# GlaireDaggers/Pretty-Fast-Video

Measured on AMD Instinct MI355X. Metric: macroblocks/s (encode+decode) 1080p YUV420, higher is better.
Workload: dtype i32 (encoder transforms evaluated in exact f32; decoders i32)

## Files before the change

### pretty-fast-video_amd/csrc/pfv_device.h

```cpp
#pragma once
#include <stdint.h>

#ifdef PFV_HIPEMU
#define PFV_WAVES_PER_EU(n)
#else
#define PFV_WAVES_PER_EU(n) __attribute__((amdgpu_waves_per_eu(n, n)))
#endif

namespace pfv {

constexpr int kStripMB = 8;
#ifndef PFV_STRIPS_PER_WG
#define PFV_STRIPS_PER_WG 4
#endif
constexpr int kStripsPerWG = PFV_STRIPS_PER_WG;
constexpr int kThreads = 64 * kStripsPerWG;

struct QTab {
    float rcp[64];
    int32_t deq[64];
};

struct PlaneGeom {
    int w, h;
    int pw, ph;
    int bw, bh;
    int strips_x;
    int strip0;
    int tiles_y;
    int tile0;
    int mb0;
    int qsel;
    int clear;
    int fast_src;
    long src_off;
    long pad_off;
};

struct FrameGeom {
    PlaneGeom p[3];
    int n_planes;
    int strips_per_frame;
    int tiles_per_frame;
    int mbs_per_frame;
    int n_streams;
    long src_frame_bytes;
    long pad_frame_bytes;
    const uint8_t *const *src_slots;
};
__host__ __device__ inline const uint8_t *frame_src(const FrameGeom &g, const uint8_t *src, int stream)
{
    return g.src_slots ? g.src_slots[stream] : src + (long)stream * g.src_frame_bytes;
}

struct CoefLists {
    const uint32_t *const *entries;
    const uint32_t *counts;
};
constexpr uint32_t coef_entry(uint32_t mb, uint32_t pos, int16_t value) { return ((uint32_t)(uint16_t)value << 16) | ((mb & 255u) << 8) | (pos & 255u); }

}
```

### pretty-fast-video_amd/csrc/pfv_kernels.hip

```cpp
#include <hip/hip_runtime.h>
#include <stdint.h>

#include "pfv_device.h"
#include "pfv_prof.h"


namespace pfv {

namespace {
__constant__ int kScale[64] = {
    32, 37, 34, 26, 32, 26, 34, 37, 37, 43, 39, 31, 37, 31, 39, 43, 34, 39, 35, 28, 34, 28, 35, 39, 26, 31, 28, 22, 26, 22,
    28, 31, 32, 37, 34, 26, 32, 26, 34, 37, 26, 31, 28, 22, 26, 22, 28, 31, 34, 39, 35, 28, 34, 28, 35, 39, 37, 43, 39, 31,
    37, 31, 39, 43,
};
__constant__ int kInvZigzag[64] = {
    0,  1,  5,  6,  14, 15, 27, 28, 2,  4,  7,  13, 16, 26, 29, 42, 3,  8,  12, 17, 25, 30, 41, 43, 9,  11, 18, 24, 31, 40,
    44, 53, 10, 19, 23, 32, 39, 45, 52, 54, 20, 22, 33, 38, 46, 51, 55, 60, 21, 34, 37, 47, 50, 56, 59, 61, 35, 36, 48, 49,
    57, 58, 62, 63,
};
}

constexpr int kWinRows = 16 * kStripsPerWG + 30;
constexpr int kWinStride = 176;
constexpr int kWinBytes = kWinRows * kWinStride;
// ... 137 lines not shown
    int a5 = wadd(wadd(wsub(b5.x, b6.x), b6.q), b6.s);
    int a6 = wsub(wsub(wadd(b6.x, b5.x), b5.q), b5.s);
    int a0 = wadd(b0, b2), a1 = wadd(b1, b3), a2 = wsub(b1, b3), a3 = wsub(b0, b2);
    v[0] = wadd(a0, a4); v[1] = wadd(a1, a5); v[2] = wadd(a2, a6); v[3] = wadd(a3, a7);
    v[4] = wsub(a3, a7); v[5] = wsub(a2, a6); v[6] = wsub(a1, a5); v[7] = wsub(a0, a4);
}

__device__ __forceinline__ void rows_to_cols2(int (&v)[2][8], int *mb, int i, int mx)
{
    const int sw = (i >> 2) & 1;
#pragma unroll
    for (int s = 0; s < 2; s++) {
        int4 *w = reinterpret_cast<int4 *>(mb + s * 64 + (i ^ mx) * 8);
        w[sw] = make_int4(v[s][0], v[s][1], v[s][2], v[s][3]);
        w[sw ^ 1] = make_int4(v[s][4], v[s][5], v[s][6], v[s][7]);
    }
    wave_lds_sync();
    const int lo = i, hi = i ^ 4;
#pragma unroll
    for (int s = 0; s < 2; s++) {
#pragma unroll
        for (int r = 0; r < 8; r++) v[s][r] = mb[s * 64 + (r ^ mx) * 8 + (r < 4 ? lo : hi)];
    }
    wave_lds_sync();
}
__device__ __forceinline__ void cols_to_rows2(int (&v)[2][8], int *mb, int i, int mx)
{
    const int lo = i, hi = i ^ 4;
#pragma unroll
    for (int s = 0; s < 2; s++) {
#pragma unroll
        for (int r = 0; r < 8; r++) mb[s * 64 + (r ^ mx) * 8 + (r < 4 ? lo : hi)] = v[s][r];
    }
    wave_lds_sync();
    const int sw = (i >> 2) & 1;
#pragma unroll
    for (int s = 0; s < 2; s++) {
        const int4 *w = reinterpret_cast<const int4 *>(mb + s * 64 + (i ^ mx) * 8);
        int4 a = w[sw], b = w[sw ^ 1];
        v[s][0] = a.x; v[s][1] = a.y; v[s][2] = a.z; v[s][3] = a.w;
        v[s][4] = b.x; v[s][5] = b.y; v[s][6] = b.z; v[s][7] = b.w;
    }
    wave_lds_sync();
}

struct LaneQ {
    const int *tab;
    int c;
    __device__ __forceinline__ float rcp(int k) const { return __int_as_float(tab[(k * 8 + c) * 4 + 0]); }
    __device__ __forceinline__ int scale(int k) const { return tab[(k * 8 + c) * 4 + 1]; }
    __device__ __forceinline__ int zz(int k) const { return tab[(k * 8 + c) * 4 + 2]; }
    __device__ __forceinline__ int deq(int k) const { return tab[(k * 8 + c) * 4 + 3]; }
    __device__ __forceinline__ float deqf(int k) const { return __int_as_float(tab[(k * 8 + c) * 4 + 3]); }
};
constexpr int kQTabDwords = 4 * 64;
template <bool ENC, bool FLT = false>
__device__ __forceinline__ int4 load_qentry(const QTab *qt, int lane)
{
    int4 e;
    e.x = ENC ? __float_as_int(qt->rcp[lane]) : 0;
    e.y = ENC ? (FLT ? (kScale[lane] << 16) : kScale[lane]) : 0;
    e.z = kInvZigzag[lane];
    e.w = FLT ? __float_as_int((float)qt->deq[lane]) : qt->deq[lane];
    return e;
}
template <bool ENC, bool FLT = false>
__device__ __forceinline__ void fill_qtable(int *tab, const QTab *qt, int lane)
{
    reinterpret_cast<int4 *>(tab)[lane] = load_qentry<ENC, FLT>(qt, lane);
}
__device__ __forceinline__ unsigned pack4(int a, int b, int c, int d)
{
    return (unsigned)a | ((unsigned)b << 8) | ((unsigned)c << 16) | ((unsigned)d << 24);
}
__device__ __forceinline__ int byte_of(unsigned w, int i) { return (int)((w >> (8 * i)) & 0xffu); }

__device__ __forceinline__ void unpack_row(const uint4 &row, int (&px)[2][8])
{
#pragma unroll
    for (int k = 0; k < 4; k++) {
        px[0][k] = byte_of(row.x, k); px[0][k + 4] = byte_of(row.y, k);
        px[1][k] = byte_of(row.z, k); px[1][k + 4] = byte_of(row.w, k);
    }
}
__device__ __forceinline__ uint4 pack_row(const int (&px)[2][8])
{
    return make_uint4(pack4(px[0][0], px[0][1], px[0][2], px[0][3]), pack4(px[0][4], px[0][5], px[0][6], px[0][7]),
                      pack4(px[1][0], px[1][1], px[1][2], px[1][3]), pack4(px[1][4], px[1][5], px[1][6], px[1][7]));
}

__device__ __forceinline__ uint4 ld_stream(const uint4 *p)
{
    return make_uint4(__builtin_nontemporal_load(&p->x), __builtin_nontemporal_load(&p->y), __builtin_nontemporal_load(&p->z),
                      __builtin_nontemporal_load(&p->w));
}
__device__ __forceinline__ void st_stream(uint4 *p, const uint4 &v)
{
    __builtin_nontemporal_store(v.x, &p->x); __builtin_nontemporal_store(v.y, &p->y);
    __builtin_nontemporal_store(v.z, &p->z); __builtin_nontemporal_store(v.w, &p->w);
}

__device__ __forceinline__ uint4 load_src16(const uint8_t *plane, const PlaneGeom &p, int x, int y)
{
    unsigned fill = (unsigned)p.clear * 0x01010101u;
    uint4 val = make_uint4(fill, fill, fill, fill);
    if (y < p.h && x < p.w) {
        const uint8_t *src = plane + (long)y * p.w + x;
        if (p.fast_src && x + 16 <= p.w) {
            val = *reinterpret_cast<const uint4 *>(src);
        } else {
            unsigned wds[4];
#pragma unroll
            for (int i = 0; i < 4; i++) {
                unsigned acc = 0;
#pragma unroll
                for (int b = 0; b < 4; b++) {
                    int xx = x + i * 4 + b;
                    unsigned px = xx < p.w ? (unsigned)src[i * 4 + b] : (unsigned)p.clear;
                    acc |= px << (8 * b);
                }
                wds[i] = acc;
            }
            val = make_uint4(wds[0], wds[1], wds[2], wds[3]);
        }
    }
    return val;
}

__device__ __forceinline__ uint4 load_unaligned16(const uint8_t *p)
{
    int sh = (int)((uintptr_t)p & 3);
    const unsigned *d = reinterpret_cast<const unsigned *>(p - sh);
    unsigned d0 = d[0], d1 = d[1], d2 = d[2], d3 = d[3], d4 = sh ? d[4] : 0u;
    return make_uint4(__builtin_amdgcn_alignbyte(d1, d0, sh), __builtin_amdgcn_alignbyte(d2, d1, sh),
                      __builtin_amdgcn_alignbyte(d3, d2, sh), __builtin_amdgcn_alignbyte(d4, d3, sh));
}

__device__ __forceinline__ void store_cropped16(uint8_t *plane, const PlaneGeom &p, int x, int y, const uint4 &val)
{
    if (y < p.h && x < p.w) st_stream(reinterpret_cast<uint4 *>(plane + (long)y * p.w + x), val);
}

typedef __attribute__((address_space(3))) void lds_void_t;
typedef __attribute__((address_space(1))) const void gbl_cvoid_t;

__device__ __forceinline__ int stage_chunk(int ch) { return (ch >> 4) * kStageChunks + (ch & 15); }
__device__ __forceinline__ void store_coef_half(const int *stage, int16_t *coef_mb0, int n_mb, int lane, int h)
{
#pragma unroll
    for (int j = 0; j < 2; j++) {
        int ch = j * 64 + lane;
        int mb = ch >> 4;
        if (mb < n_mb) st_stream(&reinterpret_cast<uint4 *>(coef_mb0)[mb * 32 + h * 16 + (ch & 15)], reinterpret_cast<const uint4 *>(stage)[stage_chunk(ch)]);
    }
}
__device__ __forceinline__ void fetch_coef_half(uint4 (&buf)[2], const int16_t *coef_mb0, int n_mb, int lane, int h)
{
#pragma unroll
    for (int j = 0; j < 2; j++) {
        int ch = j * 64 + lane;
        int mb = ch >> 4;
        buf[j] = make_uint4(0, 0, 0, 0);
        if (mb < n_mb) buf[j] = ld_stream(&reinterpret_cast<const uint4 *>(coef_mb0)[mb * 32 + h * 16 + (ch & 15)]);
    }
}
__device__ __forceinline__ void store_coef_quads(const int *stage, int16_t *coef_mb0, int n_mb, int lane, int half_strip)
{
#pragma unroll
    for (int j = 0; j < 2; j++) {
        int ch = j * 64 + lane;
        int mb = half_strip * 4 + (ch >> 5);
        if (mb < n_mb) st_stream(&reinterpret_cast<uint4 *>(coef_mb0)[half_strip * 128 + ch], reinterpret_cast<const uint4 *>(stage)[stage_chunk(ch)]);
    }
}
__device__ __forceinline__ void fetch_coef_quads(uint4 (&buf)[2], const int16_t *coef_mb0, int n_mb, int lane, int half_strip)
{
#pragma unroll
    for (int j = 0; j < 2; j++) {
        int ch = j * 64 + lane;
        int mb = half_strip * 4 + (ch >> 5);
        buf[j] = make_uint4(0, 0, 0, 0);
        if (mb < n_mb) buf[j] = ld_stream(&reinterpret_cast<const uint4 *>(coef_mb0)[half_strip * 128 + ch]);
    }
}
__device__ __forceinline__ void stage_coef_half(int *stage, const uint4 (&buf)[2], int lane)
{
#pragma unroll
    for (int j = 0; j < 2; j++) reinterpret_cast<uint4 *>(stage)[stage_chunk(j * 64 + lane)] = buf[j];
}

struct ListSpan {
    const uint32_t *ent;
    uint32_t lo, hi;
    uint32_t e0, e1;
};
__device__ __forceinline__ ListSpan list_span(const uint32_t *ent, uint32_t begin, uint32_t end, int last_lane, int lane)
{
    ListSpan sp{ent, 0u, 0u, 0u, 0u};
    sp.lo = (uint32_t)__builtin_amdgcn_readlane((int)begin, 0);
    sp.hi = (uint32_t)__builtin_amdgcn_readlane((int)end, last_lane);
    if (sp.hi < sp.lo) sp.hi = sp.lo;
    const uint32_t k = sp.lo + (uint32_t)lane;
    if (k < sp.hi) sp.e0 = ent[k];
    if (k + 64u < sp.hi) sp.e1 = ent[k + 64u];
    return sp;
}
template <int LPM>
__device__ __forceinline__ void stage_list_put(int16_t *stage, uint32_t e, int mb_low, int h)
{
    const int pos = (int)(e & 255u), mbl = (int)(((e >> 8) - (uint32_t)mb_low) & 255u);
    if (LPM == 8) {
        if ((pos >> 7) == h && mbl < kStripMB) stage[mbl * (2 * kStagePitch) + (pos & 127)] = (int16_t)(e >> 16);
    } else {
        if (mbl < kStripMB / 2) stage[(mbl * 2 + (pos >> 7)) * (2 * kStagePitch) + (pos & 127)] = (int16_t)(e >> 16);
    }
}
template <int LPM>
__device__ __forceinline__ void stage_list_half(int *xw, const ListSpan &sp, int lane, int mb_low, int h)
{
#pragma unroll
    for (int j = 0; j < 2; j++) reinterpret_cast<uint4 *>(xw)[stage_chunk(j * 64 + lane)] = make_uint4(0, 0, 0, 0);
    wave_lds_sync();
    int16_t *stage = reinterpret_cast<int16_t *>(xw);
    const uint32_t k = sp.lo + (uint32_t)lane;
    if (k < sp.hi) stage_list_put<LPM>(stage, sp.e0, mb_low, h);
    if (k + 64u < sp.hi) stage_list_put<LPM>(stage, sp.e1, mb_low, h);
    for (uint32_t j = k + 128u; j < sp.hi; j += 64u) stage_list_put<LPM>(stage, sp.ent[j], mb_low, h);
}

__device__ __forceinline__ void forward_half(int (&v)[2][8], int *xw, int m, int i, const LaneQ &lq, bool keep)
{
    const int keepmask = keep ? -1 : 0;
    int *mb = xw + m * kMBPitch;
    fdct8(v[0]);
    fdct8(v[1]);
// ... 117 lines not shown
        for (int j = 0; j < 4; j++) {
            const float4 c = row[f_chunk(p, j)];
            x[2 * j] = f2{c.x, c.y};
            x[2 * j + 1] = f2{c.z, c.w};
        }
    }
    wave_lds_sync();
}
__device__ __forceinline__ f2 quant_scale(f2 m, int scale16)
{
    f2 n;
#pragma unroll
    for (int s = 0; s < 2; s++) n[s] = (float)mulhi24((int)m[s], scale16);
    return n;
}
constexpr float kQuantMagic = 12582912.0f;
__device__ __forceinline__ f2 quant_div(f2 n, float rcp, float magic, f2 &biased)
{
    const f2 q = f2trunc(n * f2s(rcp));
    biased = q + f2s(magic);
    return q;
}
__device__ __forceinline__ f2 quant_pair_f(f2 m, int scale16, float rcp, float magic, f2 &biased)
{
    return quant_div(quant_scale(m, scale16), rcp, magic, biased);
}
__device__ __forceinline__ f2 residual_f(f2 src, f2 pred)
{
    const f2 d = src - pred;
    const float c = 0.5f - 1.0f / 2048.0f;
    const f2 r = f2{__builtin_fmaf(d[0], c, kQuantMagic), __builtin_fmaf(d[1], c, kQuantMagic)};
    return f2{__builtin_fmaf(r[0], 256.0f, -256.0f * kQuantMagic), __builtin_fmaf(r[1], 256.0f, -256.0f * kQuantMagic)};
}
__device__ __forceinline__ int16_t quant_low16(float biased) { return (int16_t)__float_as_int(biased); }
__device__ __forceinline__ void forward_half_f(f2 (&x)[8], int *xw, int m, int i, const LaneQ &lq, float magic)
{
    int *mb = xw + m * kMBPitch;
    ffdct8(x);
    f_rows_to_cols(x, mb, i, m & 3);
    ffdct8(x);
    int16_t *stage = reinterpret_cast<int16_t *>(xw) + m * (2 * kStagePitch);
#pragma unroll
    for (int k = 0; k < 8; k++) {
        const int zz = lq.zz(k);
        f2 biased;
        x[k] = quant_pair_f(x[k], lq.scale(k), lq.rcp(k), magic, biased);
#pragma unroll
        for (int s = 0; s < 2; s++) stage[s * 64 + zz] = quant_low16(biased[s]);
    }
    wave_lds_sync();
}
constexpr float kPixelBias = 127.501953125f;
__device__ __forceinline__ f2 iframe_pixel_f(f2 x) { return x * f2s(1.0f / 256.0f) + f2s(kPixelBias); }
template <bool PIXEL>
__device__ __forceinline__ void inverse_half_f(f2 (&c)[8], int *xw, int m, int i, const LaneQ &lq)
{
    int *mb = xw + m * kMBPitch;
#pragma unroll
    for (int k = 0; k < 8; k++) c[k] = c[k] * f2s(lq.deqf(k));
    fidct8(c);
    f_cols_to_rows(c, mb, i, m & 3);
    fidct8(c);
#pragma unroll
    for (int k = 0; k < 8; k++) c[k] = PIXEL ? iframe_pixel_f(c[k]) : f2floor(c[k] * f2s(1.0f / 256.0f));
}
__device__ __forceinline__ uint4 pack_row_f(const f2 (&px)[8])
{
    unsigned w[4] = {0, 0, 0, 0};
#pragma unroll
    for (int k = 0; k < 8; k++) {
        w[k >> 2] = __builtin_amdgcn_cvt_pk_u8_f32(px[k][0], (unsigned)(k & 3), w[k >> 2]);
        w[2 + (k >> 2)] = __builtin_amdgcn_cvt_pk_u8_f32(px[k][1], (unsigned)(k & 3), w[2 + (k >> 2)]);
    }
    return make_uint4(w[0], w[1], w[2], w[3]);
}
__device__ __forceinline__ void unpack_row_f(const uint4 &row, f2 (&px)[8])
{
#pragma unroll
    for (int k = 0; k < 4; k++) {
        px[k] = f2{(float)byte_of(row.x, k), (float)byte_of(row.z, k)};
        px[k + 4] = f2{(float)byte_of(row.y, k), (float)byte_of(row.w, k)};
    }
}

template <bool FLT, int LPM = 8>
__global__ __launch_bounds__(kThreads) void k_enc_iframe(FrameGeom g, const uint8_t *__restrict__ src,
                                                          int16_t *__restrict__ coef, uint8_t *__restrict__ recon,
                                                          const QTab *__restrict__ qtabs, float qmagic)
{
    __shared__ __attribute__((aligned(16))) int xchg[kStripsPerWG][kXchgDwords];
    __shared__ __attribute__((aligned(16))) int qtab_lds[kStripsPerWG][kQTabDwords];
    constexpr int kPasses = LPM == 8 ? 2 : 1;

    const int lane = threadIdx.x & 63, wave = __builtin_amdgcn_readfirstlane((int)(threadIdx.x >> 6));
    const int gw = xcd_remap((int)blockIdx.x, (int)gridDim.x) * kStripsPerWG + wave;
    const int gstrip = LPM == 8 ? gw : gw >> 1, half_strip = LPM == 8 ? 0 : gw & 1;
    if (gstrip >= g.strips_per_frame * g.n_streams) return;
    const StripPos sp = locate_strip(g, gstrip);
    if (half_strip * 4 >= sp.n_mb) return;
    const PlaneGeom &p = g.p[sp.plane];
    const int slot = lane >> 3, i = lane & 7;
    const int m = LPM == 8 ? slot : half_strip * 4 + (slot >> 1);
    int *xw = xchg[wave];

    fill_qtable<true, FLT>(qtab_lds[wave], qtabs + p.qsel, lane);
    const uint8_t *plane = frame_src(g, src, sp.stream) + p.src_off;
    uint4 rows[kPasses];
#pragma unroll
    for (int pass = 0; pass < kPasses; pass++) rows[pass] = load_src16(plane, p, sp.x0 + m * 16, sp.y0 + i + 8 * (LPM == 8 ? pass : (slot & 1)));

    wave_lds_sync();
    const LaneQ lq{qtab_lds[wave], i};
    int16_t *coef_mb0 = coef + ((long)sp.stream * g.mbs_per_frame + sp.mb_first) * 256;
    uint8_t *dst = recon ? recon + (long)sp.stream * g.pad_frame_bytes + p.pad_off + (long)(sp.y0 + i) * p.pw + sp.x0 + m * 16
                         : nullptr;
#pragma unroll
    for (int pass = 0; pass < kPasses; pass++) {
        const int h = LPM == 8 ? pass : (slot & 1);
        if (FLT) {
            f2 x[8];
            unpack_row_f(rows[pass], x);
#pragma unroll
            for (int k = 0; k < 8; k++) x[k] = x[k] * f2s(256.0f) - f2s(32768.0f);
            forward_half_f(x, xw, slot, i, lq, qmagic);
            if (LPM == 8) store_coef_half(xw, coef_mb0, sp.n_mb, lane, h);
            else store_coef_quads(xw, coef_mb0, sp.n_mb, lane, half_strip);
            wave_lds_sync();
            if (recon) {
                inverse_half_f<true>(x, xw, slot, i, lq);
                if (m < sp.n_mb) *reinterpret_cast<uint4 *>(dst + (long)(8 * h) * p.pw) = pack_row_f(x);
            }
        } else {
            int v[2][8];
            unpack_row(rows[pass], v);
#pragma unroll
// ... 286 lines not shown
    const int wrow0 = mby - tp.winy0 + i;

    unsigned s2 = 0;
#pragma unroll
    for (int h = 0; h < 2; h++) {
        s2 = __builtin_amdgcn_udot4(rows[h].x, rows[h].x, s2, false);
        s2 = __builtin_amdgcn_udot4(rows[h].y, rows[h].y, s2, false);
        s2 = __builtin_amdgcn_udot4(rows[h].z, rows[h].z, s2, false);
        s2 = __builtin_amdgcn_udot4(rows[h].w, rows[h].w, s2, false);
    }
    const int a2 = mb_sum((int)s2);

    SearchState st;
    st.cx = 0; st.cy = 0; st.err = 0;
    const SearchLane sl = make_search_lane(red, m, i, neg2);
    const bool interior = sp.x0 >= 16 && sp.x0 + kStripMB * 16 + 16 <= p.pw && sp.y0 >= 16 && sp.y0 + 32 <= p.ph;
    if (interior) {
        search_level<8, true, false, DPPRED>(win, wrow0, wcol0, rows[0], rows[1], a2, mbx, mby, p.pw, p.ph, st, sl);
        KMARK(3);
        search_level<4, false, false, DPPRED>(win, wrow0, wcol0, rows[0], rows[1], a2, mbx, mby, p.pw, p.ph, st, sl);
        KMARK(4);
        search_level<2, false, false, DPPRED>(win, wrow0, wcol0, rows[0], rows[1], a2, mbx, mby, p.pw, p.ph, st, sl);
        KMARK(5);
        search_level<1, false, false, DPPRED>(win, wrow0, wcol0, rows[0], rows[1], a2, mbx, mby, p.pw, p.ph, st, sl);
        KMARK(6);
    } else {
        search_level<8, true, true, DPPRED>(win, wrow0, wcol0, rows[0], rows[1], a2, mbx, mby, p.pw, p.ph, st, sl);
        search_level<4, false, true, DPPRED>(win, wrow0, wcol0, rows[0], rows[1], a2, mbx, mby, p.pw, p.ph, st, sl);
        search_level<2, false, true, DPPRED>(win, wrow0, wcol0, rows[0], rows[1], a2, mbx, mby, p.pw, p.ph, st, sl);
        search_level<1, false, true, DPPRED>(win, wrow0, wcol0, rows[0], rows[1], a2, mbx, mby, p.pw, p.ph, st, sl);
    }

    so.coded = mb_valid && !((float)st.err <= min_err);
    so.cx = st.cx; so.cy = st.cy;

    const int wx = wcol0 + st.cx, shp = wx & 3;
    const uint8_t *rp = win + (wrow0 + st.cy) * kWinStride + (wx & ~3);
#pragma unroll
    for (int h = 0; h < 2; h++) {
        const unsigned *d = reinterpret_cast<const unsigned *>(rp + 8 * h * kWinStride);
        unsigned d0 = d[0], d1 = d[1], d2 = d[2], d3 = d[3], d4 = d[4];
        so.patch[h] = make_uint4(__builtin_amdgcn_alignbyte(d1, d0, shp), __builtin_amdgcn_alignbyte(d2, d1, shp),
                                 __builtin_amdgcn_alignbyte(d3, d2, shp), __builtin_amdgcn_alignbyte(d4, d3, shp));
    }
}

__device__ __forceinline__ void opaque_row(uint4 &r)
{
#ifndef PFV_HIPEMU
    asm volatile("" : "+v"(r.x), "+v"(r.y), "+v"(r.z), "+v"(r.w));
#else
    (void)r;
#endif
}
template <bool FLT, bool REUNPACK = false, class Store>
__device__ __forceinline__ uint4 penc_half(const uint4 &srow, const uint4 &prow, int *xw, int m, int i, const LaneQ &lq, float qmagic, bool want_recon,
                                           Store &&store)
{
    uint4 out = prow;
    if (FLT) {
        f2 x[8], pp[8];
        unpack_row_f(srow, x);
        unpack_row_f(prow, pp);
#pragma unroll
        for (int k = 0; k < 8; k++) x[k] = residual_f(x[k], pp[k]);
        forward_half_f(x, xw, m, i, lq, qmagic);
        store();
        wave_lds_sync();
        if (want_recon) {
            inverse_half_f<false>(x, xw, m, i, lq);
            if (REUNPACK) {
                uint4 again = prow;
                opaque_row(again);
                unpack_row_f(again, pp);
            }
#pragma unroll
            for (int k = 0; k < 8; k++) {
                const f2 t = f2{__builtin_fminf(x[k][0], 127.0f), __builtin_fminf(x[k][1], 127.0f)};
                pp[k] = pp[k] + t * f2s(2.0f);
            }
            out = pack_row_f(pp);
        }
    } else {
        int v[2][8], pp[2][8];
        unpack_row(srow, v);
        unpack_row(prow, pp);
#pragma unroll
        for (int s = 0; s < 2; s++) {
#pragma unroll
            for (int k = 0; k < 8; k++) {
                int d = v[s][k] - pp[s][k];
                v[s][k] = (int)((unsigned)tdiv2(d) << 8);
            }
        }
        forward_half(v, xw, m, i, lq, true);
        store();
        wave_lds_sync();
        if (want_recon) {
            inverse_half(v, xw, m, i, lq);
#pragma unroll
            for (int s = 0; s < 2; s++) {
#pragma unroll
                for (int k = 0; k < 8; k++)
                    pp[s][k] = min(max(pp[s][k] + 2 * v[s][k], 0), 255);
            }
            out = pack_row(pp);
// ... 515 lines not shown
        if (recon && mb_valid) *reinterpret_cast<uint4 *>(dst) = o;
    } else if (mb_valid) {
        uint4 *cm = reinterpret_cast<uint4 *>(coef_mb0 + m * 256);
        st_stream(&cm[r], make_uint4(0, 0, 0, 0));
        st_stream(&cm[16 + r], make_uint4(0, 0, 0, 0));
        if (dst) *reinterpret_cast<uint4 *>(dst) = patch;
    }
}

template <int LPM = 8, bool LISTS = false>
__global__ __launch_bounds__(kThreads) void k_dec_iframe(FrameGeom g, const int16_t *__restrict__ coef, CoefLists cl,
                                                          uint8_t *__restrict__ out, const QTab *__restrict__ qtabs,
                                                          uint8_t *__restrict__ frames_out)
{
    __shared__ __attribute__((aligned(16))) int xchg[kStripsPerWG][kXchgDwords];
    __shared__ __attribute__((aligned(16))) int qtab_lds[kStripsPerWG][kQTabDwords];
    constexpr int kPasses = LPM == 8 ? 2 : 1;

    const int lane = threadIdx.x & 63, wave = __builtin_amdgcn_readfirstlane((int)(threadIdx.x >> 6));
    const int gw = xcd_remap((int)blockIdx.x, (int)gridDim.x) * kStripsPerWG + wave;
    const int gstrip = LPM == 8 ? gw : gw >> 1, half_strip = LPM == 8 ? 0 : gw & 1;
    if (gstrip >= g.strips_per_frame * g.n_streams) return;
    const StripPos sp = locate_strip(g, gstrip);
    if (half_strip * 4 >= sp.n_mb) return;
    const PlaneGeom &p = g.p[sp.plane];
    const int slot = lane >> 3, i = lane & 7;
    const int m = LPM == 8 ? slot : half_strip * 4 + (slot >> 1);
    int *xw = xchg[wave];

    const int16_t *coef_mb0 = coef + ((long)sp.stream * g.mbs_per_frame + sp.mb_first) * 256;
    uint4 cbuf[kPasses][2];
    ListSpan span;
    if (LISTS) {
        const int last = min(sp.n_mb - half_strip * 4, LPM == 8 ? 8 : 4) - 1;
        const uint32_t *cnt = cl.counts + (long)sp.stream * (g.mbs_per_frame + 1) + sp.mb_first + half_strip * 4;
        const int mw = min(LPM == 8 ? slot : (slot >> 1), last);
        span = list_span(cl.entries[sp.stream], cnt[mw], cnt[mw + 1], last * (LPM == 8 ? 8 : 16), lane);
    } else if (LPM == 8) {
        fetch_coef_half(cbuf[0], coef_mb0, sp.n_mb, lane, 0);
        fetch_coef_half(cbuf[kPasses - 1], coef_mb0, sp.n_mb, lane, 1);
    } else {
        fetch_coef_quads(cbuf[0], coef_mb0, sp.n_mb, lane, half_strip);
    }
    fill_qtable<false>(qtab_lds[wave], qtabs + p.qsel, lane);
    wave_lds_sync();
    const LaneQ lq{qtab_lds[wave], i};
    uint8_t *dst = out + (long)sp.stream * g.pad_frame_bytes + p.pad_off + (long)(sp.y0 + i) * p.pw + sp.x0 + m * 16;
#pragma unroll
    for (int pass = 0; pass < kPasses; pass++) {
        const int h = LPM == 8 ? pass : (slot & 1);
        if (LISTS) stage_list_half<LPM>(xw, span, lane, sp.mb_first + half_strip * 4, pass);
        else stage_coef_half(xw, cbuf[pass], lane);
        wave_lds_sync();
        int v[2][8];
        gather_half(v, xw, slot, lq);
        inverse_half(v, xw, slot, i, lq);
#pragma unroll
        for (int s = 0; s < 2; s++)
#pragma unroll
            for (int k = 0; k < 8; k++) v[s][k] = min(max(v[s][k] + 128, 0), 255);
        if (m < sp.n_mb) {
            const uint4 o = pack_row(v);
            *reinterpret_cast<uint4 *>(dst + (long)(8 * h) * p.pw) = o;
            if (frames_out)
                store_cropped16(frames_out + (long)sp.stream * g.src_frame_bytes + p.src_off, p, sp.x0 + m * 16, sp.y0 + i + 8 * h, o);
        }
    }
}

template <int LPM = 8, bool LISTS = false>
__global__ __launch_bounds__(kThreads) void k_dec_pframe(FrameGeom g, const int8_t *__restrict__ mv,
                                                          const uint8_t *__restrict__ has, const int16_t *__restrict__ coef, CoefLists cl,
                                                          const uint8_t *__restrict__ ref, uint8_t *__restrict__ out,
                                                          const QTab *__restrict__ qtabs, int *__restrict__ err_flag,
                                                          uint8_t *__restrict__ frames_out)
{
    __shared__ __attribute__((aligned(16))) int xchg[kStripsPerWG][kXchgDwords];
    __shared__ __attribute__((aligned(16))) int qtab_lds[kStripsPerWG][kQTabDwords];
    constexpr int kPasses = LPM == 8 ? 2 : 1;

    const int lane = threadIdx.x & 63, wave = __builtin_amdgcn_readfirstlane((int)(threadIdx.x >> 6));
    const int gw = xcd_remap((int)blockIdx.x, (int)gridDim.x) * kStripsPerWG + wave;
    const int gstrip = LPM == 8 ? gw : gw >> 1, half_strip = LPM == 8 ? 0 : gw & 1;
    if (gstrip >= g.strips_per_frame * g.n_streams) return;
    const StripPos sp = locate_strip(g, gstrip);
    if (half_strip * 4 >= sp.n_mb) return;
    const PlaneGeom &p = g.p[sp.plane];
    const int slot = lane >> 3, i = lane & 7;
    const int m = LPM == 8 ? slot : half_strip * 4 + (slot >> 1);
    int *xw = xchg[wave];
    const bool mb_valid = m < sp.n_mb;
    const long mbi = (long)sp.stream * g.mbs_per_frame + sp.mb_first + (mb_valid ? m : 0);

    int mx = mv[mbi * 2 + 0], my = mv[mbi * 2 + 1];
    const bool coded = mb_valid && has[mbi] != 0;
    uint32_t cnt0 = 0, cnt1 = 0;
    int last_mb = 0;
    if (LISTS) {
        last_mb = min(sp.n_mb - half_strip * 4, LPM == 8 ? 8 : 4) - 1;
        const uint32_t *cnt = cl.counts + (long)sp.stream * (g.mbs_per_frame + 1) + sp.mb_first + half_strip * 4;
        const int mw = min(LPM == 8 ? slot : (slot >> 1), last_mb);
        cnt0 = cnt[mw]; cnt1 = cnt[mw + 1];
    }
    fill_qtable<false>(qtab_lds[wave], qtabs + p.qsel, lane);

    const int mbx = sp.x0 + m * 16, mby = sp.y0;
    if (mb_valid) {
        int sx = mbx + mx, sy = mby + my;
        if (sx < 0 || sx > p.pw - 16 || sy < 0 || sy > p.ph - 16) {
            if (i == 0) atomicOr(err_flag + sp.stream, 1);
            mx = 0; my = 0;
        }
    }
    const bool any_coded = __any(coded);
    const int16_t *coef_mb0 = coef + ((long)sp.stream * g.mbs_per_frame + sp.mb_first) * 256;
    uint4 cbuf[kPasses][2];
    ListSpan span;
    if (any_coded) {
        if (LISTS) {
            span = list_span(cl.entries[sp.stream], cnt0, cnt1, last_mb * (LPM == 8 ? 8 : 16), lane);
        } else if (LPM == 8) {
            fetch_coef_half(cbuf[0], coef_mb0, sp.n_mb, lane, 0);
            fetch_coef_half(cbuf[kPasses - 1], coef_mb0, sp.n_mb, lane, 1);
        } else {
            fetch_coef_quads(cbuf[0], coef_mb0, sp.n_mb, lane, half_strip);
        }
    }
    uint4 patch[kPasses];
#pragma unroll
    for (int pass = 0; pass < kPasses; pass++) patch[pass] = make_uint4(0, 0, 0, 0);
    if (mb_valid) {
        const uint8_t *rp = ref + (long)sp.stream * g.pad_frame_bytes + p.pad_off + (long)(mby + my + i) * p.pw + (mbx + mx);
#pragma unroll
        for (int pass = 0; pass < kPasses; pass++) patch[pass] = load_unaligned16(rp + 8 * (long)(LPM == 8 ? pass : (slot & 1)) * p.pw);
    }
    uint8_t *dst = out + (long)sp.stream * g.pad_frame_bytes + p.pad_off + (long)(sp.y0 + i) * p.pw + mbx;
    uint8_t *crop = frames_out ? frames_out + (long)sp.stream * g.src_frame_bytes + p.src_off : nullptr;

    if (any_coded) {
        wave_lds_sync();
        const LaneQ lq{qtab_lds[wave], i};
#pragma unroll
        for (int pass = 0; pass < kPasses; pass++) {
            const int h = LPM == 8 ? pass : (slot & 1);
            if (LISTS) stage_list_half<LPM>(xw, span, lane, sp.mb_first + half_strip * 4, pass);
            else stage_coef_half(xw, cbuf[pass], lane);
            wave_lds_sync();
            int v[2][8], pp[2][8];
            const int codedmask = coded ? -1 : 0;
            gather_half(v, xw, slot, lq);
            inverse_half(v, xw, slot, i, lq);
            unpack_row(patch[pass], pp);
#pragma unroll
            for (int s = 0; s < 2; s++)
#pragma unroll
                for (int k = 0; k < 8; k++)
                    pp[s][k] = min(max(pp[s][k] + 2 * (v[s][k] & codedmask), 0), 255);
            if (mb_valid) {
                const uint4 o = pack_row(pp);
                *reinterpret_cast<uint4 *>(dst + (long)(8 * h) * p.pw) = o;
                if (crop) store_cropped16(crop, p, mbx, sp.y0 + i + 8 * h, o);
            }
        }
    } else if (mb_valid) {
#pragma unroll
        for (int pass = 0; pass < kPasses; pass++) {
            const int h = LPM == 8 ? pass : (slot & 1);
            *reinterpret_cast<uint4 *>(dst + (long)(8 * h) * p.pw) = patch[pass];
            if (crop) store_cropped16(crop, p, mbx, sp.y0 + i + 8 * h, patch[pass]);
        }
    }
}

#ifndef PFV_PENC_TU
__global__ __launch_bounds__(kThreads) void k_blit(uint8_t *__restrict__ dst, int dst_w, const uint8_t *__restrict__ src,
                                                    int src_w, int dx, int dy, int sx, int sy, int sw, int sh)
{
    long n = (long)sw * sh;
// ... 123 lines not shown
```

### pretty-fast-video_amd/csrc/pfv_launch.hip

```cpp
static float biased_rcp(int q)
{
    volatile float r = q ? 1.0f / (float)q : 0.0f;
    r = r * 1.000000476837158203125f;
    return r;
}
static int make_qtab(pfv_ctx *ctx, const int32_t q[64], QTab *out, bool decode_only = false)
{
    if (!q) return fail(ctx, PFV_ERR_BAD_ARG, "q-table is null");
    for (int i = 0; i < 64; i++)
        if (q[i] < (decode_only ? 0 : 1) || q[i] > 65535) return fail(ctx, PFV_ERR_BAD_ARG, "q-table entry outside [1,65535]");
    for (int i = 0; i < 64; i++) {
        out->rcp[i] = biased_rcp(q[i]);
        int z = H_INV_ZIGZAG[i];
        out->deq[i] = (int32_t)((uint32_t)H_SCALE[z] * (uint32_t)q[z]);
    }
    return PFV_OK;
}

static int ensure_scratch(pfv_ctx *ctx, int slot, size_t bytes, void **out)
{
    if (bytes == 0) bytes = 16;
    if (ctx->scratch_cap[slot] < bytes) {
        if (ctx->scratch[slot]) {
            HIP_TRY(ctx, hipStreamSynchronize(ctx->stream));
            HIP_TRY(ctx, hipFree(ctx->scratch[slot]));
            ctx->scratch[slot] = nullptr;
            ctx->scratch_cap[slot] = 0;
        }
        size_t cap = (bytes + 4095) & ~(size_t)4095;
        HIP_TRY(ctx, hipMalloc(&ctx->scratch[slot], cap));
        ctx->scratch_cap[slot] = cap;
    }
    *out = ctx->scratch[slot];
    return PFV_OK;
}

static void fill_plane(PlaneGeom &p, int w, int h, int strip0, int mb0, long src_off, long pad_off, int qsel, int clear)
{
    p.w = w; p.h = h;
    p.pw = pad16(w); p.ph = pad16(h);
    p.bw = p.pw / 16; p.bh = p.ph / 16;
    p.strips_x = (p.bw + kStripMB - 1) / kStripMB;
    p.tiles_y = (p.bh + kStripsPerWG - 1) / kStripsPerWG;
    p.strip0 = strip0; p.mb0 = mb0;
    p.tile0 = 0;
    p.qsel = qsel; p.clear = clear;
    p.src_off = src_off; p.pad_off = pad_off;
    p.fast_src = 0;
}

static FrameGeom plane_geom(int w, int h, int clear)
{
    FrameGeom g;
    memset(&g, 0, sizeof g);
    fill_plane(g.p[0], w, h, 0, 0, 0, 0, 0, clear);
    g.p[1] = g.p[0]; g.p[2] = g.p[0];
    g.n_planes = 1;
    g.strips_per_frame = g.p[0].strips_x * g.p[0].bh;
    g.tiles_per_frame = g.p[0].strips_x * g.p[0].tiles_y;
    g.mbs_per_frame = g.p[0].bw * g.p[0].bh;
    g.n_streams = 1;
    g.src_frame_bytes = (long)w * h;
    g.pad_frame_bytes = (long)g.p[0].pw * g.p[0].ph;
    g.p[0].fast_src = (w % 16 == 0);
    return g;
}

static FrameGeom frame_geom(int w, int h, int n_streams)
// ... 132 lines not shown
```

### pretty-fast-video_amd/csrc/pfv_sessions.hip

```cpp
static int init_padded(pfv_ctx *ctx, const FrameGeom &g, uint8_t *buf)
{
    dim3 grid(64, 3, g.n_streams);
    hipLaunchKernelGGL(k_init_padded, grid, dim3(kThreads), 0, ctx->stream, g, buf);
    return launch_check(ctx, "k_init_padded");
}

struct XformNorms {
    double F1[8];
    double Iabs[8][8];
    signed char fsign[64];
    signed char isign[64];
};
static const XformNorms &xform_norms()
{
    static const XformNorms t = [] {
        XformNorms n{};
        for (int k = 0; k < 8; k++) {
            int f[8] = {0, 0, 0, 0, 0, 0, 0, 0}, i8[8] = {0, 0, 0, 0, 0, 0, 0, 0};
            f[k] = i8[k] = 1 << 20;
            fdct8(f);
            idct8(i8);
            for (int u = 0; u < 8; u++) {
                n.F1[u] += fabs((double)f[u]) / (1 << 20);
                n.Iabs[u][k] = fabs((double)i8[u]) / (1 << 20);
                n.fsign[u * 8 + k] = (signed char)(f[u] < 0 ? -1 : 1);
                n.isign[u * 8 + k] = (signed char)(i8[u] < 0 ? -1 : 1);
            }
        }
        return n;
    }();
    return t;
}
static double enc_max_coef(const int32_t q[64], double amplitude, int i)
{
    const XformNorms &n = xform_norms();
    const double M = amplitude * n.F1[i >> 3] * n.F1[i & 7];
    return floor(floor(M * H_SCALE[i] / 65536.0) / (double)q[i]);
}
static bool enc_float_exact(const int32_t q[64], double amplitude)
{
    const XformNorms &nm = xform_norms();
    double D[8][8], worst = 0;
    for (int i = 0; i < 64; i++) {
        const int u = i >> 3, v = i & 7, z = H_INV_ZIGZAG[i];
        const double M = amplitude * nm.F1[u] * nm.F1[v];
        const double c = enc_max_coef(q, amplitude, i);
        D[u][v] = c * (double)H_SCALE[z] * (double)q[z];
        worst = std::max(worst, std::max(M, D[u][v]));
    }
    double col[8][8];
    for (int u = 0; u < 8; u++)
        for (int v = 0; v < 8; v++) {
            double a = 16;
            for (int k = 0; k < 8; k++) a += nm.Iabs[u][k] * D[k][v];
            col[u][v] = a;
            worst = std::max(worst, a);
        }
    for (int u = 0; u < 8; u++)
        for (int v = 0; v < 8; v++) {
            double a = 16;
            for (int k = 0; k < 8; k++) a += col[u][k] * nm.Iabs[v][k];
            worst = std::max(worst, a);
        }
    return worst < 8388608.0;
}

struct pfv_enc_session {
    pfv_ctx *ctx = nullptr;
    int width = 0, height = 0, n_streams = 0;
    FrameGeom geom;
    QTab *qtab_dev = nullptr;
    float px_err = 0.0f;
    bool flt = false;
    int tile_compaction = 1;
    int lane_mapping = PFV_LANES_AUTO;
    uint8_t *prev[2] = {nullptr, nullptr};
    int cur = 0;
    int win_first = 0, win_count = 0;
    size_t in_stride = 0;
    uint8_t *st_frames = nullptr;
    int16_t *st_coef = nullptr;
    int8_t *st_mv = nullptr;
    uint8_t *st_has = nullptr;
    bool ent_on = false;
    uint32_t ent_cap = 0;
    EntBufs ent{};
    std::vector<void *> ent_allocs;
    std::vector<uint32_t> ent_sizes;
    uint8_t *ent_packed = nullptr;
    uint32_t *ent_offsets_dev = nullptr;
    size_t ent_packed_cap = 0;
    hipStream_t ent_stream = nullptr;
    hipEvent_t ev_encoded = nullptr;
    hipEvent_t ev_packed[2] = {nullptr, nullptr};
    int ev_cur = 0;
    bool ev_prev_valid = false;
};

struct pfv_dec_session {
    pfv_ctx *ctx = nullptr;
    int width = 0, height = 0, n_streams = 0, n_qtables = 0;
    FrameGeom geom;
    QTab *qtab_dev = nullptr;
    uint8_t *fb[2] = {nullptr, nullptr};
    int lane_mapping = PFV_LANES_AUTO;
    int cur = 0;
    int *flag_dev = nullptr;
    std::vector<int> flags_host;
    uint8_t *frames_out = nullptr;
    size_t out_stride = 0;
    int win_first = 0, win_count = 0;
    int16_t *st_coef = nullptr;
    int8_t *st_mv = nullptr;
    uint8_t *st_has = nullptr;
    uint8_t *st_frames = nullptr;
    uint32_t *st_idx = nullptr;
    int16_t *st_val = nullptr;
// ... 774 lines not shown
```

Before: 1.438 billion.

## Use guarded float inverse DCT in decoder and skip fetching uncoded coefficients

The decoder's intra path now gathers coefficients as floats and checks them against per-coefficient limits computed on the host from a worst-case bound on the inverse transform's intermediates. When every lane is within bounds it runs a float IDCT, otherwise it falls back to the exact integer path. Coefficient fetches are also masked by a ballot of coded macroblocks, so uncoded blocks cause no global loads. The cost is an extra gather and reduction per half, a divergent fallback path, added register pressure, and reliance on the host bound to keep results bit-exact.

```diff
diff --git a/pretty-fast-video_amd/csrc/pfv_device.h b/pretty-fast-video_amd/csrc/pfv_device.h
--- a/pretty-fast-video_amd/csrc/pfv_device.h
+++ b/pretty-fast-video_amd/csrc/pfv_device.h
@@ -19,6 +19,7 @@
 struct QTab {
     float rcp[64];
     int32_t deq[64];
+    float dlim[64];
 };
 
 struct PlaneGeom {
diff --git a/pretty-fast-video_amd/csrc/pfv_kernels.hip b/pretty-fast-video_amd/csrc/pfv_kernels.hip
--- a/pretty-fast-video_amd/csrc/pfv_kernels.hip
+++ b/pretty-fast-video_amd/csrc/pfv_kernels.hip
@@ -213,14 +213,16 @@
     __device__ __forceinline__ int zz(int k) const { return tab[(k * 8 + c) * 4 + 2]; }
     __device__ __forceinline__ int deq(int k) const { return tab[(k * 8 + c) * 4 + 3]; }
     __device__ __forceinline__ float deqf(int k) const { return __int_as_float(tab[(k * 8 + c) * 4 + 3]); }
+    __device__ __forceinline__ float dlim(int k) const { return __int_as_float(tab[(k * 8 + c) * 4 + 0]); }
+    __device__ __forceinline__ float ddeqf(int k) const { return __int_as_float(tab[(k * 8 + c) * 4 + 1]); }
 };
 constexpr int kQTabDwords = 4 * 64;
 template <bool ENC, bool FLT = false>
 __device__ __forceinline__ int4 load_qentry(const QTab *qt, int lane)
 {
     int4 e;
-    e.x = ENC ? __float_as_int(qt->rcp[lane]) : 0;
-    e.y = ENC ? (FLT ? (kScale[lane] << 16) : kScale[lane]) : 0;
+    e.x = __float_as_int(ENC ? qt->rcp[lane] : qt->dlim[lane]);
+    e.y = ENC ? (FLT ? (kScale[lane] << 16) : kScale[lane]) : __float_as_int((float)qt->deq[lane]);
     e.z = kInvZigzag[lane];
     e.w = FLT ? __float_as_int((float)qt->deq[lane]) : qt->deq[lane];
     return e;
@@ -315,14 +317,14 @@
         if (mb < n_mb) st_stream(&reinterpret_cast<uint4 *>(coef_mb0)[mb * 32 + h * 16 + (ch & 15)], reinterpret_cast<const uint4 *>(stage)[stage_chunk(ch)]);
     }
 }
-__device__ __forceinline__ void fetch_coef_half(uint4 (&buf)[2], const int16_t *coef_mb0, int n_mb, int lane, int h)
+__device__ __forceinline__ void fetch_coef_half(uint4 (&buf)[2], const int16_t *coef_mb0, int n_mb, int lane, int h, unsigned long long want = ~0ull)
 {
 #pragma unroll
     for (int j = 0; j < 2; j++) {
         int ch = j * 64 + lane;
         int mb = ch >> 4;
         buf[j] = make_uint4(0, 0, 0, 0);
-        if (mb < n_mb) buf[j] = ld_stream(&reinterpret_cast<const uint4 *>(coef_mb0)[mb * 32 + h * 16 + (ch & 15)]);
+        if (mb < n_mb && ((want >> (8 * mb)) & 1)) buf[j] = ld_stream(&reinterpret_cast<const uint4 *>(coef_mb0)[mb * 32 + h * 16 + (ch & 15)]);
     }
 }
 __device__ __forceinline__ void store_coef_quads(const int *stage, int16_t *coef_mb0, int n_mb, int lane, int half_strip)
@@ -334,14 +336,15 @@
         if (mb < n_mb) st_stream(&reinterpret_cast<uint4 *>(coef_mb0)[half_strip * 128 + ch], reinterpret_cast<const uint4 *>(stage)[stage_chunk(ch)]);
     }
 }
-__device__ __forceinline__ void fetch_coef_quads(uint4 (&buf)[2], const int16_t *coef_mb0, int n_mb, int lane, int half_strip)
+__device__ __forceinline__ void fetch_coef_quads(uint4 (&buf)[2], const int16_t *coef_mb0, int n_mb, int lane, int half_strip,
+                                                 unsigned long long want = ~0ull)
 {
 #pragma unroll
     for (int j = 0; j < 2; j++) {
         int ch = j * 64 + lane;
         int mb = half_strip * 4 + (ch >> 5);
         buf[j] = make_uint4(0, 0, 0, 0);
-        if (mb < n_mb) buf[j] = ld_stream(&reinterpret_cast<const uint4 *>(coef_mb0)[half_strip * 128 + ch]);
+        if (mb < n_mb && ((want >> (16 * (ch >> 5))) & 1)) buf[j] = ld_stream(&reinterpret_cast<const uint4 *>(coef_mb0)[half_strip * 128 + ch]);
     }
 }
 __device__ __forceinline__ void stage_coef_half(int *stage, const uint4 (&buf)[2], int lane)
@@ -565,12 +568,12 @@
 }
 constexpr float kPixelBias = 127.501953125f;
 __device__ __forceinline__ f2 iframe_pixel_f(f2 x) { return x * f2s(1.0f / 256.0f) + f2s(kPixelBias); }
-template <bool PIXEL>
+template <bool PIXEL, bool DEC = false>
 __device__ __forceinline__ void inverse_half_f(f2 (&c)[8], int *xw, int m, int i, const LaneQ &lq)
 {
     int *mb = xw + m * kMBPitch;
 #pragma unroll
-    for (int k = 0; k < 8; k++) c[k] = c[k] * f2s(lq.deqf(k));
+    for (int k = 0; k < 8; k++) c[k] = c[k] * f2s(DEC ? lq.ddeqf(k) : lq.deqf(k));
     fidct8(c);
     f_cols_to_rows(c, mb, i, m & 3);
     fidct8(c);
@@ -594,6 +597,20 @@
         px[k] = f2{(float)byte_of(row.x, k), (float)byte_of(row.z, k)};
         px[k + 4] = f2{(float)byte_of(row.y, k), (float)byte_of(row.w, k)};
     }
+}
+__device__ __forceinline__ bool gather_half_f(f2 (&x)[8], const int *xw, int m, const LaneQ &lq)
+{
+    const int16_t *stage = reinterpret_cast<const int16_t *>(xw) + m * (2 * kStagePitch);
+    float w = 0.0f;
+#pragma unroll
+    for (int k = 0; k < 8; k++) {
+        const int zz = lq.zz(k);
+        x[k] = f2{(float)stage[zz], (float)stage[64 + zz]};
+        const f2 y = x[k] * f2s(lq.dlim(k));
+        w = __builtin_fmaxf(w, __builtin_fmaxf(__builtin_fabsf(y[0]), __builtin_fabsf(y[1])));
+    }
+    wave_lds_sync();
+    return !__any(!(w <= 1.0f));
 }
 
 template <bool FLT, int LPM = 8>
@@ -986,6 +1003,13 @@
 #else
     (void)r;
 #endif
+}
+__device__ __forceinline__ int opaque_int(int x)
+{
+#ifndef PFV_HIPEMU
+    asm volatile("" : "+v"(x));
+#endif
+    return x;
 }
 template <bool FLT, bool REUNPACK = false, class Store>
 __device__ __forceinline__ uint4 penc_half(const uint4 &srow, const uint4 &prow, int *xw, int m, int i, const LaneQ &lq, float qmagic, bool want_recon,
@@ -1607,15 +1631,23 @@
         if (LISTS) stage_list_half<LPM>(xw, span, lane, sp.mb_first + half_strip * 4, pass);
         else stage_coef_half(xw, cbuf[pass], lane);
         wave_lds_sync();
-        int v[2][8];
-        gather_half(v, xw, slot, lq);
-        inverse_half(v, xw, slot, i, lq);
-#pragma unroll
-        for (int s = 0; s < 2; s++)
-#pragma unroll
-            for (int k = 0; k < 8; k++) v[s][k] = min(max(v[s][k] + 128, 0), 255);
+        f2 x[8];
+        uint4 o;
+        const int ps = opaque_int(slot), pi = opaque_int(i);
+        if (gather_half_f(x, xw, ps, lq)) {
+            inverse_half_f<true, true>(x, xw, ps, pi, lq);
+            o = pack_row_f(x);
+        } else {
+            int v[2][8];
+            gather_half(v, xw, ps, lq);
+            inverse_half(v, xw, ps, pi, lq);
+#pragma unroll
+            for (int s = 0; s < 2; s++)
+#pragma unroll
+                for (int k = 0; k < 8; k++) v[s][k] = min(max(v[s][k] + 128, 0), 255);
+            o = pack_row(v);
+        }
         if (m < sp.n_mb) {
-            const uint4 o = pack_row(v);
             *reinterpret_cast<uint4 *>(dst + (long)(8 * h) * p.pw) = o;
             if (frames_out)
                 store_cropped16(frames_out + (long)sp.stream * g.src_frame_bytes + p.src_off, p, sp.x0 + m * 16, sp.y0 + i + 8 * h, o);
@@ -1667,7 +1699,8 @@
             mx = 0; my = 0;
         }
     }
-    const bool any_coded = __any(coded);
+    const unsigned long long coded_bits = __ballot(coded);
+    const bool any_coded = coded_bits != 0;
     const int16_t *coef_mb0 = coef + ((long)sp.stream * g.mbs_per_frame + sp.mb_first) * 256;
     uint4 cbuf[kPasses][2];
     ListSpan span;
@@ -1675,10 +1708,10 @@
         if (LISTS) {
             span = list_span(cl.entries[sp.stream], cnt0, cnt1, last_mb * (LPM == 8 ? 8 : 16), lane);
         } else if (LPM == 8) {
-            fetch_coef_half(cbuf[0], coef_mb0, sp.n_mb, lane, 0);
-            fetch_coef_half(cbuf[kPasses - 1], coef_mb0, sp.n_mb, lane, 1);
+            fetch_coef_half(cbuf[0], coef_mb0, sp.n_mb, lane, 0, coded_bits);
+            fetch_coef_half(cbuf[kPasses - 1], coef_mb0, sp.n_mb, lane, 1, coded_bits);
         } else {
-            fetch_coef_quads(cbuf[0], coef_mb0, sp.n_mb, lane, half_strip);
+            fetch_coef_quads(cbuf[0], coef_mb0, sp.n_mb, lane, half_strip, coded_bits);
         }
     }
     uint4 patch[kPasses];
diff --git a/pretty-fast-video_amd/csrc/pfv_launch.hip b/pretty-fast-video_amd/csrc/pfv_launch.hip
--- a/pretty-fast-video_amd/csrc/pfv_launch.hip
+++ b/pretty-fast-video_amd/csrc/pfv_launch.hip
@@ -4,6 +4,7 @@
     r = r * 1.000000476837158203125f;
     return r;
 }
+static void dec_guard_limits(const int32_t q[64], float dlim[64]);
 static int make_qtab(pfv_ctx *ctx, const int32_t q[64], QTab *out, bool decode_only = false)
 {
     if (!q) return fail(ctx, PFV_ERR_BAD_ARG, "q-table is null");
@@ -14,6 +15,7 @@
         int z = H_INV_ZIGZAG[i];
         out->deq[i] = (int32_t)((uint32_t)H_SCALE[z] * (uint32_t)q[z]);
     }
+    dec_guard_limits(q, out->dlim);
     return PFV_OK;
 }
 
diff --git a/pretty-fast-video_amd/csrc/pfv_sessions.hip b/pretty-fast-video_amd/csrc/pfv_sessions.hip
--- a/pretty-fast-video_amd/csrc/pfv_sessions.hip
+++ b/pretty-fast-video_amd/csrc/pfv_sessions.hip
@@ -63,6 +63,52 @@
             worst = std::max(worst, a);
         }
     return worst < 8388608.0;
+}
+
+static double idct8_bound(double (&v)[8])
+{
+    const double c0 = v[0], d4 = v[1], c2 = v[2], d6 = v[3], c1 = v[4], d5 = v[5], c3 = v[6], d7 = v[7];
+    const double c5 = d5 + d6, c7 = d5 + d6;
+    const double b4 = d4 + c5, b5 = d4 + c5, b6 = d7 + c7, b7 = d7 + c7;
+    const double b0 = c0 + c1, b1 = c0 + c1;
+    const double b2 = c2 + c2 / 4 + c3 / 2, b3 = c2 / 2 + c3 + c3 / 4;
+    const double a4 = b7 / 4 + b4 + b4 / 4 + b4 / 16, a7 = b4 / 4 + b7 + b7 / 4 + b7 / 16;
+    const double a5 = b5 + b6 + b6 / 4 + b6 / 16, a6 = b6 + b5 + b5 / 4 + b5 / 16;
+    const double a0 = b0 + b2, a1 = b1 + b3, a2 = b1 + b3, a3 = b0 + b2;
+    v[0] = a0 + a4; v[1] = a1 + a5; v[2] = a2 + a6; v[3] = a3 + a7;
+    v[4] = a3 + a7; v[5] = a2 + a6; v[6] = a1 + a5; v[7] = a0 + a4;
+    double worst = 0;
+    for (double x : {c0, d4, c2, d6, c1, d5, c3, d7, c5, b4, b6, b0, b2, b3, a4, a5, a6, a7, a0, a1, v[0], v[1], v[2], v[3]}) worst = std::max(worst, x);
+    return worst;
+}
+static void dec_guard_limits(const int32_t q[64], float dlim[64])
+{
+    const XformNorms &nm = xform_norms();
+    const double amplitude = 128.0 * 256.0;
+    double lim[64], D[8][8], worst = 0;
+    bool ok = true;
+    for (int i = 0; i < 64; i++) {
+        if (q[i] <= 0) { ok = false; break; }
+        const int z = H_INV_ZIGZAG[i];
+        const double M = amplitude * nm.F1[i >> 3] * nm.F1[i & 7];
+        lim[i] = std::min(floor(ceil(M * H_SCALE[i] / 65536.0) / (double)q[i]), 32768.0);
+        D[i >> 3][i & 7] = lim[i] * (double)H_SCALE[z] * (double)q[z];
+        worst = std::max(worst, D[i >> 3][i & 7]);
+    }
+    for (int c = 0; ok && c < 8; c++) {
+        double v[8];
+        for (int k = 0; k < 8; k++) v[k] = D[k][c];
+        worst = std::max(worst, idct8_bound(v));
+        for (int k = 0; k < 8; k++) D[k][c] = v[k];
+    }
+    for (int r = 0; ok && r < 8; r++) worst = std::max(worst, idct8_bound(D[r]));
+    ok = ok && worst < 16777216.0;
+    for (int i = 0; i < 64; i++) {
+        if (!ok || lim[i] < 1) { dlim[i] = 0x1p100f; continue; }
+        float r = (float)(1.0 / lim[i]);
+        if ((double)r > 1.0 / lim[i]) r = nextafterf(r, 0.0f);
+        dlim[i] = r;
+    }
 }
 
 struct pfv_enc_session {
```

Result: no change. 1.433 billion (median of 2 runs) (-0.4%).
